# mrankitvish/ai-agent-kubectl

Measured on AMD Instinct MI355X. Metric: requests/sec + p50 e2e latency, /kubectl-command Llama-3-8B 1/2/4/8 GPU, higher is better.
Workload: dtype bf16; 1 GPU; model=Llama-3-8B-Instruct, global_batch=256, seq_len=115, parallelism=dp1

## Files before the change

ai_agent_kubectl_amd/csrc/attention.hip:

```cpp
#include "common.h"

#define HD 128
#define KBS 16


struct DecodeFuse {
  const bf16_t* qkv;
  const float* P;
  int split;
  int pbf16;
  size_t pstride;
  const int* positions;
  const float* cos_sin;
  const int* slot_mapping;
  bf16_t* k_cache;
  bf16_t* v_cache;
  const int* nshared;
  bf16_t* q_out;
  float* part_o;
  float* part_ml;
};

constexpr int DQ_UNROLL = 4;
template <int N>
__device__ __forceinline__ void dq_ld4n(const DecodeFuse& f, const size_t (&off)[N], const bool (&en)[N],
                                        uint2 (&out)[N]) {
  if (f.P == nullptr) {
#pragma unroll
    for (int n = 0; n < N; ++n)
      if (en[n]) out[n] = *reinterpret_cast<const uint2*>(f.qkv + off[n]);
    return;
  }
  f32x4 s[N];
#pragma unroll
  for (int n = 0; n < N; ++n) s[n] = f32x4{0.f, 0.f, 0.f, 0.f};
  if (f.pbf16) {
    const bf16_t* pb = reinterpret_cast<const bf16_t*>(f.P);
    for (int k0 = 0; k0 < f.split; k0 += DQ_UNROLL) {
      uint2 q[DQ_UNROLL][N];
#pragma unroll
      for (int k = 0; k < DQ_UNROLL; ++k)
#pragma unroll
        for (int n = 0; n < N; ++n)
          if (en[n] && k0 + k < f.split) q[k][n] = *reinterpret_cast<const uint2*>(pb + (k0 + k) * f.pstride + off[n]);
#pragma unroll
      for (int k = 0; k < DQ_UNROLL; ++k)
#pragma unroll
        for (int n = 0; n < N; ++n)
          if (en[n] && k0 + k < f.split) s[n] += f32x4{lo_f(q[k][n].x), hi_f(q[k][n].x), lo_f(q[k][n].y), hi_f(q[k][n].y)};
    }
  } else {
    constexpr int U = DQ_UNROLL / 2;
    for (int k0 = 0; k0 < f.split; k0 += U) {
      f32x4 p[U][N];
#pragma unroll
      for (int k = 0; k < U; ++k)
#pragma unroll
        for (int n = 0; n < N; ++n)
          if (en[n] && k0 + k < f.split) p[k][n] = *reinterpret_cast<const f32x4*>(f.P + (k0 + k) * f.pstride + off[n]);
#pragma unroll
      for (int k = 0; k < U; ++k)
#pragma unroll
        for (int n = 0; n < N; ++n)
          if (en[n] && k0 + k < f.split) s[n] += p[k][n];
    }
  }
#pragma unroll
  for (int n = 0; n < N; ++n) out[n] = make_uint2(pack2(s[n][0], s[n][1]), pack2(s[n][2], s[n][3]));
}

template <bool FUSED, int NW = 4>
__global__ __launch_bounds__(64 * NW, 4) void paged_decode_kernel(bf16_t* __restrict__ out, const bf16_t* __restrict__ q,
                                                           const bf16_t* __restrict__ k_cache,
                                                           const bf16_t* __restrict__ v_cache,
                                                           const int* __restrict__ block_tables, int max_blocks,
                                                           const int* __restrict__ ctx_lens, int hq, int hkv,
                                                           float scale_log2, DecodeFuse fz) {
  const int h = blockIdx.x, b = blockIdx.y;
  const int G = hq / hkv;
  const int lane = threadIdx.x & 63, wave = FUSED ? __builtin_amdgcn_readfirstlane(threadIdx.x >> 6) : threadIdx.x >> 6;
  const int col = lane & 15, grp = lane >> 4;
  int ns = 0;
  int pos_b = 0, slot_b = -1;
// ... 537 lines not shown
    l[r] = 0.f;
  }
#pragma unroll
  for (int n = 0; n < 8; ++n) o[n] = f32x4{0.f, 0.f, 0.f, 0.f};

  u32x4 kreg[2], vreg[2];
  prefill_load_tile(kreg, vreg, k_cache, v_cache, bt, nblocks, 0, h, hkv);
  bf16_t* pw = s.p[wave];
  for (int t = 0; t < ntiles; ++t) {
    __syncthreads();
    prefill_store_tile(s, kreg, vreg);
    __syncthreads();
    if (t + 1 < ntiles) prefill_load_tile(kreg, vreg, k_cache, v_cache, bt, nblocks, t + 1, h, hkv);
    const int t0 = t * 32;
    f32x4 sc[2];
#pragma unroll
    for (int j = 0; j < 2; ++j) {
      const int tok = 16 * j + col;
      f32x4 acc = {0.f, 0.f, 0.f, 0.f};
#pragma unroll
      for (int ks = 0; ks < 4; ++ks) {
        const uint4 kf = s.k[tok][(4 * ks + grp) ^ (tok & 15)];
        acc = mfma16x16x32(qf[ks], as_bf16x8(kf), acc);
      }
      sc[j] = acc;
    }
    float alpha[4];
#pragma unroll
    for (int r = 0; r < 4; ++r) {
      const float x0 = (t0 + col <= qpos[r]) ? sc[0][r] * scale_log2 : -INFINITY;
      const float x1 = (t0 + 16 + col <= qpos[r]) ? sc[1][r] * scale_log2 : -INFINITY;
      const float mx = row16_max(fmaxf(x0, x1));
      const float mn = fmaxf(m[r], mx);
      alpha[r] = (mn == -INFINITY) ? 1.f : exp2f(m[r] - mn);
      const float p0 = (mn == -INFINITY) ? 0.f : exp2f(x0 - mn);
      const float p1 = (mn == -INFINITY) ? 0.f : exp2f(x1 - mn);
      l[r] = l[r] * alpha[r] + row16_sum(p0 + p1);
      m[r] = mn;
      p_store(pw, 4 * grp + r, col, p0, p1);
    }
#pragma unroll
    for (int n = 0; n < 8; ++n) {
#pragma unroll
      for (int r = 0; r < 4; ++r) o[n][r] *= alpha[r];
    }
    asm volatile("s_waitcnt lgkmcnt(0)" ::: "memory");
    const bf16x8 pf = p_load(pw, col, grp);
#pragma unroll
    for (int n = 0; n < 8; ++n) {
      const int dim = n * 16 + col;
      const uint4 vf = s.v[dim][grp ^ (((dim >> 2) & 1) << 1)];
      o[n] = mfma16x16x32(pf, as_bf16x8(vf), o[n]);
    }
  }
#pragma unroll
  for (int r = 0; r < 4; ++r) {
    const int row = wave * 16 + 4 * grp + r;
    const int tok = tile_tok0 + row / G;
    const int g = row % G;
    if (tok >= qlen) continue;
    const float inv = l[r] > 0.f ? 1.f / l[r] : 0.f;
    bf16_t* op = out + ((size_t)(q0 + tok) * hq + h * G + g) * HD + col;
#pragma unroll
    for (int n = 0; n < 8; ++n) op[n * 16] = f2bf(o[n][r] * inv);
  }
}

extern "C" int ka_paged_prefill(void* out, const void* q, const void* k_cache, const void* v_cache,
                                const int* block_tables, int max_blocks, const int* q_starts, const int* ctx_lens,
                                int num_seqs, int max_q_len, int hq, int hkv, int head_dim, int block_size,
                                float scale, hipStream_t stream) {
  if (num_seqs <= 0 || max_q_len <= 0) return 0;
  const int G = hkv > 0 ? hq / hkv : 0;
  if (head_dim != HD || block_size != KBS || hq % hkv != 0 || G > 64 || 64 % G != 0) return (int)hipErrorInvalidValue;
  const float scale_log2 = scale * 1.4426950408889634f;
  const int tpt = 64 / G;
  const int qtiles = (max_q_len + tpt - 1) / tpt;
  hipLaunchKernelGGL(paged_prefill_kernel, dim3(qtiles, hkv, num_seqs), dim3(256), 0, stream,
                     static_cast<bf16_t*>(out), static_cast<const bf16_t*>(q), static_cast<const bf16_t*>(k_cache),
                     static_cast<const bf16_t*>(v_cache), block_tables, max_blocks, q_starts, ctx_lens, hq, hkv,
                     scale_log2);
  KA_CHECK_LAUNCH();
}
```

ai_agent_kubectl_amd/models/llama.py:

```python
from __future__ import annotations

import os
from dataclasses import dataclass
from typing import Dict, Optional

import torch
import torch.nn.functional as F

from .. import ops
from ..parallel.comm import LocalComm
from .config import ModelConfig
from .moe import moe_forward


def persistent_default() -> bool:
    mode = os.environ.get("KA_PERSISTENT_DECODE", "auto")
    if mode in ("0", "1"):
        return mode == "1"
    return float(os.environ.get("KA_GPU_MEM_SHARE", "1")) >= 1.0


@dataclass
class AttnMeta:
    positions: torch.Tensor
    slot_mapping: torch.Tensor
    block_tables: torch.Tensor
    ctx_lens: torch.Tensor
    logits_indices: torch.Tensor
    is_decode: bool
    q_starts: Optional[torch.Tensor] = None
    max_q_len: int = 1
    num_decode: int = 0
    num_tokens: int = 0
    shared_blocks: Optional[torch.Tensor] = None


SAMP_WORDS = 6


@dataclass
class SampleArrays:
    temperature: torch.Tensor
    top_k: torch.Tensor
    top_p: torch.Tensor
    seed: torch.Tensor
    position: torch.Tensor

    @classmethod
    def from_image(cls, img: torch.Tensor, cap: int, n: int) -> "SampleArrays":
        return cls(temperature=img[0:n].view(torch.float32), top_k=img[cap:cap + n],
                   top_p=img[2 * cap:2 * cap + n].view(torch.float32), position=img[3 * cap:3 * cap + n],
                   seed=img[4 * cap:4 * cap + 2 * n].view(torch.int64))


class LlamaModel:
    def __init__(self, cfg: ModelConfig, weights: Dict[str, torch.Tensor], comm=None, tp_rank: int = 0,
                 tp_size: int = 1, ep_rank: int = 0, ep_size: int = 1):
        self.cfg = cfg
        self.W = weights
        self.comm = comm or LocalComm()
        self.tp_rank, self.tp_size = tp_rank, tp_size
        self._local_comm = isinstance(self.comm, LocalComm)
        self.ep_rank, self.ep_size = ep_rank, ep_size
        self.hq = cfg.num_heads // tp_size
        self.hkv = cfg.num_kv_heads // tp_size
        self.D = cfg.head_dim
        self.scale = cfg.head_dim ** -0.5
        self.vocab_local = weights["lm_head"].shape[0]
        self.vocab_offset = tp_rank * self.vocab_local
        dev = weights["embed"].device
        self.device = dev
        self.cos_sin = ops.rope_cos_sin(cfg.max_position, cfg.head_dim, cfg.rope_theta, device=dev)
        self.fuse_decode_rope = os.environ.get("KA_FUSE_DECODE_ROPE", "1") == "1"
        self.bf16_partials = os.environ.get("KA_BF16_PARTIALS", "1") == "1"
        self.bf16_qkv_partials = os.environ.get("KA_BF16_QKV_PARTIALS", "1") == "1"
        self.layers = [self._layer(i) for i in range(cfg.num_layers)]
        w13 = self.layers[0].get("w13") if self.layers else None
        self.i_local = w13.shape[-2] // 2 if w13 is not None else cfg.intermediate // tp_size
        self.prune_last_layer = os.environ.get("KA_PRUNE_LAST_LAYER", "1") == "1"
        self.mark_layer = -1
        self.mark_event = None
        self.prefetch_bytes = int(float(os.environ.get("KA_DECODE_PREFETCH_MB", "0")) * (1 << 20))
        self.prefetch_max_b = int(os.environ.get("KA_DECODE_PREFETCH_MAX_B", "4"))
        self.prefetch_blocks = int(os.environ.get("KA_DECODE_PREFETCH_BLOCKS", "64"))
        self._side = None
        self.persistent = persistent_default()
        self._pd = None
        self.persistent_max_b = int(os.environ.get("KA_PERSISTENT_MAX_B", "2"))
        self._pd_max_b = None
        self.persistent_stamps = None

    def _layer(self, i):
        p = f"layers.{i}."
        return {k: self.W[p + k] for k in ("wqkv", "wo", "ln1", "ln2", "w13", "w2", "router") if p + k in self.W}

    def forward(self, input_ids: torch.Tensor, meta: AttnMeta, k_cache: torch.Tensor,
                v_cache: torch.Tensor) -> torch.Tensor:
        cfg = self.cfg
        eps = cfg.norm_eps
        h = ops.embedding(input_ids, self.W["embed"])
        if ops.reference_fp32():
            h = h.float()
        if meta.is_decode and not ops._ref(h) and self.persistent_ok(input_ids.shape[0]):
            return self._forward_persistent(h, meta, k_cache, v_cache)
        residual = None
        pending = False
        T = input_ids.shape[0]
        mark = self.mark_layer
        last_li = len(self.layers) - 1
        pruned = False
        for li, L in enumerate(self.layers):
            if li == mark and input_ids.is_cuda:
                self.mark_event = torch.cuda.Event()
                self.mark_event.record()
            if residual is None:
                residual = h
                x = ops.rmsnorm(h, L["ln1"], eps)
            else:
                x = self._reduce_norm(h, L["ln1"], eps, residual, pending)
            fused = meta.is_decode and self.fuse_decode_rope
            qkv = ops.linear(x, L["wqkv"], defer_reduce=True, bf16_partials=fused and self.bf16_qkv_partials)
            side = self._fork_prefetch(L, T) if meta.is_decode else None
            if fused:
                a = ops.decode_attention_rope(qkv, meta.positions, self.cos_sin, meta.slot_mapping, k_cache[li],
                                              v_cache[li], meta.block_tables, meta.ctx_lens, self.hq, self.hkv,
                                              self.D, self.scale, shared_blocks=meta.shared_blocks)
            else:
                q = ops.rope_kv_write(qkv, meta.positions, self.cos_sin, meta.slot_mapping, k_cache[li],
                                      v_cache[li], self.hq, self.hkv, self.D)
                if li == last_li and not meta.is_decode and self.prune_last_layer:
                    idx = meta.logits_indices
                    a = ops.attention_decode(q.index_select(0, idx), k_cache[li], v_cache[li], meta.block_tables,
                                             meta.ctx_lens, self.scale)
                    residual = residual.index_select(0, idx)
                    pruned = True
                else:
                    a = self._attention(q, meta, k_cache[li], v_cache[li])
            if 0 < meta.num_tokens < T and not meta.is_decode and not pruned:
                a[meta.num_tokens:].zero_()
            fuse = self._local_comm or (meta.is_decode and getattr(self.comm, "splitk_norm", False))
            h = ops.linear(a.reshape(a.shape[0], self.hq * self.D), L["wo"], defer_reduce=fuse,
                           bf16_partials=self.bf16_partials)
            x = self._reduce_norm(h, L["ln2"], eps, residual, True)
            if side is not None:
                torch.cuda.current_stream(self.device).wait_stream(side)
            combined = False
            if cfg.is_moe:
                h, combined = moe_forward(x, L, cfg, self.ep_rank, self.ep_size, meta.is_decode, self.comm)
            elif ops.use_prefill_swiglu(x, L["w13"]):
                h = ops.linear(ops.linear_swiglu(x, L["w13"]), L["w2"], defer_reduce=fuse,
                               bf16_partials=self.bf16_partials)
            elif sw := ops.decode_swiglu_cfg(x, L["w13"]):
                h = ops.linear(ops.linear_gm_swiglu(x, L["w13"], sw), L["w2"], defer_reduce=fuse,
                               bf16_partials=self.bf16_partials)
            else:
                h = ops.swiglu_linear(ops.linear(x, L["w13"], defer_reduce=True), L["w2"], defer_reduce=fuse,
                                      bf16_partials=self.bf16_partials)
            pending = not combined
        if meta.is_decode:
            return self._reduce_norm(h, self.W["norm"], eps, residual, pending)
        if pending and not self._local_comm:
            self.comm.all_reduce(h)
        if pruned:
            return ops.rmsnorm(h, self.W["norm"], eps, residual=residual)
        if isinstance(h, ops.SplitK):
            x = ops.rmsnorm(h, self.W["norm"], eps, residual=residual)
            return x.index_select(0, meta.logits_indices)
        idx = meta.logits_indices
        return ops.rmsnorm(h.index_select(0, idx), self.W["norm"], eps, residual=residual.index_select(0, idx))

    def persistent_ok(self, B: int = 1) -> bool:
        cfg = self.cfg
        comm_ok = (self._local_comm or getattr(self.comm, "persistent_no_reduce", False)
                   or self._tp_exchange() is not None)
        I = self.i_local
        if not (self.persistent and self.device.type == "cuda" and comm_ok and not cfg.is_moe
                and self.D == 128 and self.hq % self.hkv == 0 and self.hq // self.hkv <= 8
                and cfg.hidden % 512 == 0 and I % 512 == 0 and (self.hq * self.D) % 512 == 0
                and cfg.hidden <= 16384 and 1 <= B <= self.persistent_max_b):
            return False
        if self._pd_max_b is None:
            self._pd_max_b = ops.decode_persistent_max_b(cfg.hidden, self.hq, I, self.hq // self.hkv)
        return B <= self._pd_max_b

    def _tp_exchange(self):
        car = getattr(self.comm, "custom_ar", None)
        if car is None or self.tp_size <= 1 or os.environ.get("KA_PERSISTENT_TP", "0") != "1":
            return None
        return car.pd_exchange()

    def _forward_persistent(self, h0, meta: AttnMeta, k_cache, v_cache) -> torch.Tensor:
        if self._pd is None:
            ptrs = [[L[k].data_ptr() for k in ("wqkv", "wo", "w13", "w2", "ln1", "ln2")] for L in self.layers]
            table = torch.tensor(ptrs, dtype=torch.int64, device=self.device)
            lib = ops._hip.require()
            ws = torch.zeros(int(lib.ka_decode_persistent_ws(self.cfg.hidden, self.hq, self.hkv, self.i_local)),
                             dtype=torch.uint8, device=self.device)
            self._pd = (table, ws)
        table, ws = self._pd
        assert k_cache.shape[3] == 16, "persistent decode needs KV block 16"
        hout = ops.decode_persistent(h0, table, len(self.layers), self.hq, self.hkv, self.i_local,
                                     self.cfg.norm_eps, self.scale, k_cache, v_cache, meta.positions,
                                     meta.slot_mapping, meta.block_tables, meta.ctx_lens, self.cos_sin, ws,
                                     self.persistent_stamps, tp=self._tp_exchange())
        return ops.rmsnorm(hout, self.W["norm"], self.cfg.norm_eps)

    def persistent_err_word(self) -> Optional[torch.Tensor]:
        if self._pd is None:
            return None
        off = int(ops._hip.require().ka_decode_persistent_err_offset())
        return self._pd[1][off:off + 4].view(torch.int32)

    def persistent_err(self) -> int:
        if self._pd is None:
            return 0
        return int(ops._hip.require().ka_decode_persistent_err(self._pd[1].data_ptr(), ops._stream()))

    def _fork_prefetch(self, L, T: int):
        if not self.prefetch_bytes or T > self.prefetch_max_b or not self.device.type == "cuda" or "w13" not in L:
            return None
        if self._side is None:
# ... 47 lines not shown
```

ai_agent_kubectl_amd/ops/__init__.py:

```python
from __future__ import annotations

import bisect
import os
from typing import NamedTuple, Optional, Tuple

import torch

from . import reference as ref
from ._hip import check, require


_FORCE_REF = False
_REF_FP32 = False


class force_reference:

    def __init__(self, fp32: bool = False):
        self.fp32 = fp32

    def __enter__(self):
        global _FORCE_REF, _REF_FP32
        self._old = (_FORCE_REF, _REF_FP32)
        _FORCE_REF, _REF_FP32 = True, self.fp32
# ... 94 lines not shown
        return q_out
    if _ref(qkv):
        return ref.rope_kv_write(qkv, positions, cos_sin, slot_mapping, k_cache, v_cache, hq, hkv, d)
    lib = require()
    T = qkv.shape[0]
    q_out = torch.empty((T, hq, d), dtype=qkv.dtype, device=qkv.device) if q_out is None else q_out
    check(lib.ka_rope_kv(_p(q_out), _p(k_cache), _p(v_cache), _p(qkv), _p(positions), _p(cos_sin),
                         _p(slot_mapping), T, hq, hkv, d, k_cache.shape[2], _stream()), "rope_kv")
    return q_out


def attention_prefill(q, k_cache, v_cache, block_tables, q_starts, ctx_lens, max_q_len: int, scale: float,
                      out: Optional[torch.Tensor] = None) -> torch.Tensor:
    if _ref(q):
        r = ref.attention_prefill(q, k_cache, v_cache, block_tables, q_starts, ctx_lens, scale)
        if out is None:
            return r
        for i in range(ctx_lens.shape[0]):
            out[int(q_starts[i]):int(q_starts[i + 1])] = r[int(q_starts[i]):int(q_starts[i + 1])]
        return out
    lib = require()
    out = torch.empty_like(q) if out is None else out
    S = ctx_lens.shape[0]
    check(lib.ka_paged_prefill(_p(out), _p(q), _p(k_cache), _p(v_cache), _p(block_tables), block_tables.shape[1],
                               _p(q_starts), _p(ctx_lens), S, int(max_q_len), q.shape[1], k_cache.shape[1],
                               q.shape[2], k_cache.shape[2], float(scale), _stream()), "paged_prefill")
    return out


def attention_decode(q, k_cache, v_cache, block_tables, ctx_lens, scale: float,
                     out: Optional[torch.Tensor] = None) -> torch.Tensor:
    if _ref(q):
        r = ref.attention_decode(q, k_cache, v_cache, block_tables, ctx_lens, scale)
        if out is None:
            return r
        out.copy_(r)
        return out
    lib = require()
    out = torch.empty_like(q) if out is None else out
    check(lib.ka_paged_decode(_p(out), _p(q), _p(k_cache), _p(v_cache), _p(block_tables), block_tables.shape[1],
                              _p(ctx_lens), q.shape[0], q.shape[1], k_cache.shape[1], q.shape[2], k_cache.shape[2],
                              float(scale), _stream()), "paged_decode")
    return out


_CASCADE_WS = {}


def cascade_ok(B: int, hq: int, hkv: int) -> bool:
    g = hq // hkv
    return hq % hkv == 0 and g in (1, 2, 4, 8)


def decode_attention_rope(qkv, positions, cos_sin, slot_mapping, k_cache, v_cache, block_tables, ctx_lens,
                          hq: int, hkv: int, d: int, scale: float, out: Optional[torch.Tensor] = None,
                          shared_blocks: Optional[torch.Tensor] = None) -> torch.Tensor:
    lead = qkv.P if isinstance(qkv, SplitK) else qkv
    if _ref(lead) or d != 128 or k_cache.shape[2] != 16 or hq % hkv or hq // hkv > 15:
        if isinstance(qkv, SplitK) and qkv.is_bf16:
            qkv = qkv.resolve()
        q = rope_kv_write(qkv, positions, cos_sin, slot_mapping, k_cache, v_cache, hq, hkv, d)
        return attention_decode(q, k_cache, v_cache, block_tables, ctx_lens, scale, out=out)
    lib = require()
    B = ctx_lens.shape[0]
    out = torch.empty((B, hq, d), dtype=k_cache.dtype, device=k_cache.device) if out is None else out
    if isinstance(qkv, SplitK):
        src, P, split, pb = None, _p(qkv.P), qkv.split, int(qkv.is_bf16)
    else:
        src, P, split, pb = _p(qkv), None, 1, 0
    if shared_blocks is not None and cascade_ok(B, hq, hkv):
        key = (k_cache.device, B, hq)
        ws = _CASCADE_WS.get(key)
        if ws is None:
            ws = torch.empty(int(lib.ka_decode_cascade_ws(B, hq)), dtype=torch.uint8, device=k_cache.device)
            _CASCADE_WS[key] = ws
        check(lib.ka_paged_decode_rope_cascade(_p(out), src, P, split, pb, _p(k_cache), _p(v_cache), _p(positions),
                                               _p(cos_sin), _p(slot_mapping), _p(block_tables), block_tables.shape[1],
                                               _p(ctx_lens), B, hq, hkv, d, k_cache.shape[2], float(scale),
                                               _p(shared_blocks), _p(ws), _stream()), "paged_decode_rope_cascade")
        return out
    check(lib.ka_paged_decode_rope(_p(out), src, P, split, pb, _p(k_cache), _p(v_cache), _p(positions), _p(cos_sin),
                                   _p(slot_mapping), _p(block_tables), block_tables.shape[1], _p(ctx_lens), B, hq,
                                   hkv, d, k_cache.shape[2], float(scale), _stream()), "paged_decode_rope")
    return out


def silu_mul(gu, out: Optional[torch.Tensor] = None) -> torch.Tensor:
    if isinstance(gu, SplitK):
        lib = require()
        gu = gu.fp32()
        T, two_i = gu.shape
        out = torch.empty((T, two_i // 2), dtype=torch.bfloat16, device=gu.P.device) if out is None else out
        check(lib.ka_silu_mul_splitk(_p(out), _p(gu.P), gu.split, T, two_i // 2, _stream()), "silu_mul_splitk")
        return out
    if _ref(gu):
        return ref.silu_mul(gu)
    lib = require()
    T, two_i = gu.shape
    out = torch.empty((T, two_i // 2), dtype=gu.dtype, device=gu.device) if out is None else out
    check(lib.ka_silu_mul(_p(out), _p(gu), T, two_i // 2, _stream()), "silu_mul")
    return out


def prefetch(t: torch.Tensor, nbytes: int = 0, blocks: int = 0) -> None:
    if _ref(t):
        return
    lib = require()
    n = t.numel() * t.element_size()
    n = min(n, nbytes) if nbytes > 0 else n
    check(lib.ka_prefetch(_p(t), n, int(blocks), None, _stream()), "prefetch")


def embedding(ids: torch.Tensor, table: torch.Tensor, vocab_offset: int = 0,
              out: Optional[torch.Tensor] = None) -> torch.Tensor:
    if _ref(table):
        return ref.embedding(ids, table, vocab_offset)
    lib = require()
    T = ids.shape[0]
    out = torch.empty((T, table.shape[1]), dtype=table.dtype, device=table.device) if out is None else out
    check(lib.ka_embedding(_p(out), _p(ids), _p(table), T, table.shape[1], table.shape[0], int(vocab_offset),
                           _stream()), "embedding")
    return out


def masked_argmax(logits: torch.Tensor, mask_bits: Optional[torch.Tensor], mask_idx: Optional[torch.Tensor],
                  vocab_offset: int = 0, out_idx: Optional[torch.Tensor] = None,
                  out_val: Optional[torch.Tensor] = None) -> Tuple[torch.Tensor, torch.Tensor]:
    if _ref(logits):
        return ref.masked_argmax(logits, mask_bits, mask_idx, vocab_offset)
    lib = require()
    B, V = logits.shape
    out_idx = torch.empty(B, dtype=torch.int32, device=logits.device) if out_idx is None else out_idx
    out_val = torch.empty(B, dtype=torch.float32, device=logits.device) if out_val is None else out_val
    words = mask_bits.shape[1] if mask_bits is not None else 0
    slices = lib.ka_argmax_slices(B, V)
    ws = torch.empty(2 * B * slices, dtype=torch.float32, device=logits.device) if slices > 1 else None
    check(lib.ka_masked_argmax(_p(out_idx), _p(out_val), _p(logits), _p(mask_bits),
                               _p(mask_idx) if mask_bits is not None else None, B, V, words, int(vocab_offset),
                               _p(ws), slices, _stream()), "masked_argmax")
    return out_idx, out_val


def sample(logits: torch.Tensor, mask_bits: Optional[torch.Tensor], mask_idx: Optional[torch.Tensor],
           temperature: torch.Tensor, top_k: torch.Tensor, top_p: torch.Tensor, seed: torch.Tensor,
           position: torch.Tensor, vocab_offset: int = 0, return_cut: bool = False):
    if _ref(logits):
        return ref.sample(logits, mask_bits, mask_idx, temperature, top_k, top_p, seed, position, vocab_offset,
                          return_cut=return_cut)
    lib = require()
    B, V = logits.shape
    dev = logits.device
    for name, t, dt in (("temperature", temperature, torch.float32), ("top_k", top_k, torch.int32),
                        ("top_p", top_p, torch.float32), ("seed", seed, torch.int64),
                        ("position", position, torch.int32)):
        if t is None or t.dtype != dt or t.shape != (B,) or t.device != dev or not t.is_contiguous():
            raise ValueError(f"sample: {name} must be a contiguous {dt} [{B}] tensor on {dev}")
    if not logits.is_contiguous() or logits.dtype != torch.bfloat16:
        raise ValueError("sample: logits must be contiguous bf16 [rows, vocab]")
    out_idx = torch.empty(B, dtype=torch.int32, device=dev)
    out_val = torch.empty(B, dtype=torch.float32, device=dev)
    cut = torch.empty(B, dtype=torch.float32, device=dev) if return_cut else None
    kept = torch.empty(B, dtype=torch.int32, device=dev) if return_cut else None
    words = mask_bits.shape[1] if mask_bits is not None else 0
    slices = lib.ka_argmax_slices(B, V)
    ws = (torch.empty(lib.ka_sample_ws_words(B, slices), dtype=torch.int32, device=dev) if slices > 1 else None)
    check(lib.ka_sample(_p(out_idx), _p(out_val), _p(cut), _p(kept), _p(logits), _p(mask_bits),
# ... 528 lines not shown
```

ai_agent_kubectl_amd/ops/_hip.py:

```python
from __future__ import annotations

import ctypes
import os
import threading
from typing import Optional

LIB_DIR = os.path.join(os.path.dirname(os.path.abspath(__file__)), "lib")
DEFAULT_LIB = os.path.join(LIB_DIR, "libkagent_hip.so")


def _lib_path() -> str:
    alt = os.environ.get("KA_HIP_LIB")
    if alt and os.environ.get("KA_HIP_LIB_DIAG") == "1":
        return alt
    if alt:
        raise RuntimeError("KA_HIP_LIB is set without KA_HIP_LIB_DIAG=1: refusing to load a non-default "
                           f"kernel library ({alt}); unset it, or set KA_HIP_LIB_DIAG=1 for a diagnostic run")
    return DEFAULT_LIB


LIB_PATH = _lib_path()

_lock = threading.Lock()
_lib: Optional[ctypes.CDLL] = None
_err: Optional[str] = None

P = ctypes.c_void_p
I = ctypes.c_int
F = ctypes.c_float

_RESTYPES = {"ka_gemm_big_ws_bytes": ctypes.c_size_t, "ka_decode_persistent_ws": ctypes.c_size_t,
             "ka_decode_persistent_xbytes": ctypes.c_size_t, "ka_decode_persistent_xflag_offset": ctypes.c_size_t,
             "ka_decode_cascade_ws": ctypes.c_size_t}

_SIGS = {
    "ka_rmsnorm": [P, P, P, P, I, I, F, P],
    "ka_rope_kv": [P, P, P, P, P, P, P, I, I, I, I, I, P],
    "ka_silu_mul": [P, P, I, I, P],
    "ka_embedding": [P, P, P, I, I, I, I, P],
    "ka_masked_argmax": [P, P, P, P, P, I, I, I, I, P, I, P],
    "ka_argmax_slices": [I, I],
    "ka_sample": [P, P, P, P, P, P, P, P, P, P, P, P, I, I, I, I, P, I, P],
    "ka_sample_ws_words": [I, I],
    "ka_moe_topk": [P, P, P, I, I, I, P],
    "ka_paged_decode": [P, P, P, P, P, I, P, I, I, I, I, I, F, P],
    "ka_paged_decode_rope": [P, P, P, I, I, P, P, P, P, P, P, I, P, I, I, I, I, I, F, P],
    "ka_paged_decode_rope_cascade": [P, P, P, I, I, P, P, P, P, P, P, I, P, I, I, I, I, I, F, P, P, P],
    "ka_decode_cascade_ws": [I, I],
    "ka_paged_prefill": [P, P, P, P, P, I, P, P, I, I, I, I, I, I, F, P],
    "ka_gemm_skinny": [P, P, P, P, I, I, I, I, P],
    "ka_gemv_swiglu": [P, P, P, P, I, I, I, I, P],
    "ka_rmsnorm_splitk": [P, P, P, I, I, P, I, I, F, P],
    "ka_rope_kv_splitk": [P, P, P, P, I, P, P, P, I, I, I, I, I, P],
    "ka_silu_mul_splitk": [P, P, I, I, I, P],
    "ka_kv_block_copy": [P, P, P, P, I, I, ctypes.c_long, ctypes.c_long, P],
    "ka_prefetch": [P, ctypes.c_long, I, P, P],
    "ka_gemm_mfma": [P, P, P, P, I, I, I, I, I, I, I, I, I, P],
    "ka_gemv_rows": [P, P, P, P, I, I, I, I, I, I, P],
    "ka_gemm_mfma_swiglu": [P, P, P, I, I, I, I, I, I, P],
    "ka_gemm_mfma_grouped": [P, P, P, P, P, P, I, I, I, I, I, I, I, I, I, I, I, P],
    "ka_gemm_big": [P, P, P, P, I, I, I, I, I, I, I, P, ctypes.c_size_t, P],
    "ka_gemm_big_ws_bytes": [],
    "ka_gemm_big_plan": [I, I, I, I, ctypes.c_size_t, P, P],
    "ka_gemm_big_tn": [I, I, I],
    "ka_gemm_big_grouped": [P, P, P, P, I, P, I, I, I, I, I, I, I, P],
    "ka_gemm_big_err": [P, P],
    "ka_gemm_big_argmax": [P, P, P, P, I, I, I, I, P, P, I, I, P, P],
    "ka_argmax_finish": [P, P, P, P, I, I, I, P],
    "ka_argmax_combine": [P, P, P, I, I, P],
    "ka_decode_persistent": [P, P, P, I, I, I, I, I, F, F, P, P, ctypes.c_long, P, P, P, P, P, P, P, I, I, P],
    "ka_decode_persistent_tp": [P, P, P, I, I, I, I, I, F, F, P, P, ctypes.c_long, P, P, P, P, P, P, P, I, I, I, I,
                                P, P, P, P],
    "ka_decode_persistent_xbytes": [],
    "ka_decode_persistent_xflag_offset": [],
    "ka_decode_persistent_max_b": [I, I, I],
    "ka_decode_persistent_max_b2": [I, I, I, I],
    "ka_decode_persistent_ws": [I, I, I, I],
    "ka_decode_persistent_err": [P, P],
    "ka_decode_persistent_err_offset": [],
    "ka_gm_bn": [I],
    "ka_gm_bm": [I],
    "ka_moe_align": [P, P, P, I, I, I, P],
    "ka_moe_gemm": [P, P, P, P, P, I, I, I, I, I, I, I, P, P],
    "ka_moe_combine": [P, P, P, I, P, P, I, I, I, I, I, P],
    "ka_moe_sort": [P, P, P, P, P, P, I, I, I, I, I, P],
    "ka_allreduce_oneshot": [P, P, P, P, P, P, P, I, I, I, I, I, P],
    "ka_allgather_oneshot": [P, P, P, P, P, P, P, I, I, I, I, I, P],
    "ka_allreduce_rmsnorm": [P, P, P, P, F, P, P, P, P, P, I, I, I, I, I, I, I, I, P],
    "ka_ar_alloc": [P, ctypes.c_size_t],
    "ka_ar_free": [P],
    "ka_ar_get_handle": [P, P],
    "ka_ar_open_handle": [P, P],
    "ka_ar_close_handle": [P],
}


def load(path: str = LIB_PATH) -> Optional[ctypes.CDLL]:
    global _lib, _err
    with _lock:
        if _lib is not None:
            return _lib
        if not os.path.exists(path):
            _err = f"HIP kernel library not built: {path} (run python -c 'import __graft_entry__ as g; g.build()')"
            return None
        try:
            lib = ctypes.CDLL(path, mode=ctypes.RTLD_GLOBAL)
        except OSError as e:
            _err = f"failed to load {path}: {e}"
            return None
        for name, argtypes in _SIGS.items():
            fn = getattr(lib, name, None)
            if fn is None:
                continue
            fn.argtypes = argtypes
            fn.restype = _RESTYPES.get(name, ctypes.c_int)
        _lib = lib
        return _lib


def require() -> ctypes.CDLL:
    lib = load()
    if lib is None:
        raise RuntimeError(_err or "HIP kernel library unavailable")
    return lib


def available() -> bool:
    return load() is not None


def check(code: int, what: str) -> None:
    if code != 0:
# ... 2 lines not shown
```

Baseline: 1388 req/s.

## Fuse RoPE, KV-cache write and pad zeroing into paged prefill attention

Adds a paged prefill attention kernel that reads Q/K/V straight from the QKV projection output. It applies RoPE in registers, takes the new-token K/V from the activations rather than the cache, and writes the rotated K and the V into the paged cache from the first q-tile. Extra grid slices zero the padding rows, so a separate rope_kv_write kernel and a zero_ launch are no longer needed per prefill layer. The cost is a much more complex kernel: the KV-cache write is serialised in qt==0 workgroups, and the partial-tile/DPP V-transpose paths are easy to get wrong.

```diff
diff --git a/ai_agent_kubectl_amd/csrc/attention.hip b/ai_agent_kubectl_amd/csrc/attention.hip
--- a/ai_agent_kubectl_amd/csrc/attention.hip
+++ b/ai_agent_kubectl_amd/csrc/attention.hip
@@ -1,4 +1,6 @@
 #include "common.h"
+
+#include <algorithm>
 
 #define HD 128
 #define KBS 16
@@ -702,3 +704,360 @@
                      scale_log2);
   KA_CHECK_LAUNCH();
 }
+
+struct PrefillFuse {
+  const bf16_t* qkv;
+  const int* positions;
+  const float* cos_sin;
+  const int* slot_mapping;
+  bf16_t* k_cache;
+  bf16_t* v_cache;
+  int num_seqs;
+  int num_tokens;
+  int total_tokens;
+};
+
+KA_DEV void rope8(const uint4& a, const uint4& b, const float4& c0, const float4& c1, const float4& s0,
+                  const float4& s1, uint4& r1, uint4& r2) {
+  const uint32_t aw[4] = {a.x, a.y, a.z, a.w}, bw[4] = {b.x, b.y, b.z, b.w};
+  const float cc[8] = {c0.x, c0.y, c0.z, c0.w, c1.x, c1.y, c1.z, c1.w};
+  const float ss[8] = {s0.x, s0.y, s0.z, s0.w, s1.x, s1.y, s1.z, s1.w};
+  uint32_t o1[4], o2[4];
+  {
+#pragma clang fp contract(off)
+#pragma unroll
+    for (int k = 0; k < 4; ++k) {
+      const float xa0 = lo_f(aw[k]), xa1 = hi_f(aw[k]), xb0 = lo_f(bw[k]), xb1 = hi_f(bw[k]);
+      const float n0 = xb0 * ss[2 * k], n1 = xb1 * ss[2 * k + 1], p0 = xa0 * ss[2 * k], p1 = xa1 * ss[2 * k + 1];
+      o1[k] = pack2(__builtin_fmaf(xa0, cc[2 * k], -n0), __builtin_fmaf(xa1, cc[2 * k + 1], -n1));
+      o2[k] = pack2(__builtin_fmaf(xb0, cc[2 * k], p0), __builtin_fmaf(xb1, cc[2 * k + 1], p1));
+    }
+  }
+  r1 = make_uint4(o1[0], o1[1], o1[2], o1[3]);
+  r2 = make_uint4(o2[0], o2[1], o2[2], o2[3]);
+}
+
+KA_DEV uint4 rope_chunk(const uint4& own, const uint4& partner, int ch, const float4& c0, const float4& c1,
+                        const float4& s0, const float4& s1) {
+  const bool first = ch < 8;
+  uint4 r1, r2;
+  rope8(first ? own : partner, first ? partner : own, c0, c1, s0, s1, r1, r2);
+  return first ? r1 : r2;
+}
+
+KA_DEV uint32_t bf16_elem(const uint4& v, int k) {
+  const uint32_t w = (k >> 1) == 0 ? v.x : (k >> 1) == 1 ? v.y : (k >> 1) == 2 ? v.z : v.w;
+  return (k & 1) ? w >> 16 : w & 0xffffu;
+}
+
+__global__ __launch_bounds__(256, 3) void paged_prefill_rope_kernel(bf16_t* __restrict__ out,
+                                                                 const bf16_t* k_cache, const bf16_t* v_cache,
+                                                                 const int* __restrict__ block_tables, int max_blocks,
+                                                                 const int* __restrict__ q_starts,
+                                                                 const int* __restrict__ ctx_lens, int hq, int hkv,
+                                                                 float scale_log2, PrefillFuse fz) {
+  const int qt = blockIdx.x, h = blockIdx.y, sq = blockIdx.z;
+  const int tid = threadIdx.x;
+  if (sq >= fz.num_seqs) {
+    const size_t first = (size_t)fz.num_tokens * hq * (HD / 8);
+    const size_t end = (size_t)fz.total_tokens * hq * (HD / 8);
+    const size_t wg = ((size_t)(sq - fz.num_seqs) * gridDim.y + h) * gridDim.x + qt;
+    const size_t step = (size_t)(gridDim.z - fz.num_seqs) * gridDim.y * gridDim.x * 256;
+    for (size_t i = first + wg * 256 + tid; i < end; i += step)
+      reinterpret_cast<uint4*>(out)[i] = make_uint4(0, 0, 0, 0);
+    return;
+  }
+  const int G = hq / hkv;
+  const int tpt = 64 / G;
+  const int q0 = q_starts[sq];
+  const int qlen = q_starts[sq + 1] - q0;
+  const int tile_tok0 = qt * tpt;
+  if (tile_tok0 >= qlen) return;
+  const int ctx = ctx_lens[sq];
+  const int base_pos = ctx - qlen;
+  const int last_tok = min(tile_tok0 + tpt, qlen) - 1;
+  const int kv_end = base_pos + last_tok + 1;
+  const int ntiles = (kv_end + 31) >> 5;
+  const int nblocks = (ctx + KBS - 1) / KBS;
+  const int* bt = block_tables + (size_t)sq * max_blocks;
+  const size_t qstride = (size_t)(hq + 2 * hkv) * HD;
+  const size_t head_stride = (size_t)KBS * HD;
+
+  const int lane = tid & 63, wave = tid >> 6;
+  const int col = lane & 15, grp = lane >> 4;
+  __shared__ PrefillSmem s;
+
+  bf16x8 qf[4];
+  {
+    const int row = wave * 16 + col;
+    const int tok = tile_tok0 + row / G;
+    const int g = row % G;
+    if (tok < qlen) {
+      const bf16_t* qp = fz.qkv + (size_t)(q0 + tok) * qstride + (size_t)(h * G + g) * HD + 8 * grp;
+      const float* cs = fz.cos_sin + (size_t)fz.positions[q0 + tok] * HD + 8 * grp;
+      uint4 x[4];
+#pragma unroll
+      for (int ks = 0; ks < 4; ++ks) x[ks] = *reinterpret_cast<const uint4*>(qp + 32 * ks);
+#pragma unroll
+      for (int kk = 0; kk < 2; ++kk) {
+        const float* c = cs + 32 * kk;
+        uint4 r1, r2;
+        rope8(x[kk], x[kk + 2], *reinterpret_cast<const float4*>(c), *reinterpret_cast<const float4*>(c + 4),
+              *reinterpret_cast<const float4*>(c + HD / 2), *reinterpret_cast<const float4*>(c + HD / 2 + 4), r1, r2);
+        qf[kk] = as_bf16x8(r1);
+        qf[kk + 2] = as_bf16x8(r2);
+      }
+    } else {
+#pragma unroll
+      for (int ks = 0; ks < 4; ++ks) qf[ks] = as_bf16x8(make_uint4(0, 0, 0, 0));
+    }
+  }
+  int qpos[4];
+#pragma unroll
+  for (int r = 0; r < 4; ++r) {
+    const int row = wave * 16 + 4 * grp + r;
+    const int tok = tile_tok0 + row / G;
+    qpos[r] = tok < qlen ? base_pos + tok : kv_end - 1;
+  }
+  float m[4], l[4];
+  f32x4 o[8];
+#pragma unroll
+  for (int r = 0; r < 4; ++r) {
+    m[r] = -INFINITY;
+    l[r] = 0.f;
+  }
+#pragma unroll
+  for (int n = 0; n < 8; ++n) o[n] = f32x4{0.f, 0.f, 0.f, 0.f};
+
+  const int kt = tid >> 3, kc = tid & 7;
+  const int vt = tid & 31, vc = tid >> 5;
+  u32x4 kreg[2], vreg[2];
+  uint4 nv[2];
+  float4 ncs[4];
+  auto load_cache = [&](int tile) {
+    const int t0 = tile * 32;
+    if (t0 >= base_pos) return;
+    const int i0 = 2 * tile < nblocks ? 2 * tile : 0, i1 = 2 * tile + 1 < nblocks ? 2 * tile + 1 : 0;
+    const int blk0 = bt[__builtin_amdgcn_readfirstlane(i0)], blk1 = bt[__builtin_amdgcn_readfirstlane(i1)];
+    if (t0 + kt < base_pos) {
+      const bf16_t* kp = k_cache + ((size_t)((kt >> 4) ? blk1 : blk0) * hkv + h) * head_stride + (kt & 15) * HD + kc * 8;
+      kreg[0] = *reinterpret_cast<const u32x4*>(kp);
+      kreg[1] = *reinterpret_cast<const u32x4*>(kp + HD / 2);
+    }
+#pragma unroll
+    for (int i = 0; i < 2; ++i) {
+      const int p = tid + 256 * i;
+      const int dim = p >> 2, ch = p & 3;
+      const int blk = (ch >> 1) ? blk1 : blk0;
+      if (t0 + ch * 8 < base_pos)
+        vreg[i] = *reinterpret_cast<const u32x4*>(v_cache + ((size_t)blk * hkv + h) * head_stride + dim * KBS + (ch & 1) * 8);
+    }
+  };
+  auto load_new = [&](int tile) {
+    const int t0 = tile * 32;
+    if (t0 + 32 <= base_pos) return;
+    const int kpos = t0 + kt, vpos = t0 + vt;
+    if (kpos >= base_pos && kpos < ctx) {
+      const int t = q0 + kpos - base_pos;
+      const bf16_t* kp = fz.qkv + (size_t)t * qstride + (size_t)(hq + h) * HD + kc * 8;
+      kreg[0] = *reinterpret_cast<const u32x4*>(kp);
+      kreg[1] = *reinterpret_cast<const u32x4*>(kp + HD / 2);
+      const float* cs = fz.cos_sin + (size_t)fz.positions[t] * HD + kc * 8;
+      ncs[0] = *reinterpret_cast<const float4*>(cs);
+      ncs[1] = *reinterpret_cast<const float4*>(cs + 4);
+      ncs[2] = *reinterpret_cast<const float4*>(cs + HD / 2);
+      ncs[3] = *reinterpret_cast<const float4*>(cs + HD / 2 + 4);
+    }
+    if (vpos >= base_pos && vpos < ctx) {
+      const bf16_t* vp = fz.qkv + (size_t)(q0 + vpos - base_pos) * qstride + (size_t)(hq + hkv + h) * HD + vc * 8;
+      nv[0] = *reinterpret_cast<const uint4*>(vp);
+      nv[1] = *reinterpret_cast<const uint4*>(vp + HD / 2);
+    }
+  };
+  auto store_tile = [&](int tile) {
+    const int t0 = tile * 32;
+    {
+      const int kpos = t0 + kt;
+      uint4 k0 = __builtin_bit_cast(uint4, kreg[0]), k1 = __builtin_bit_cast(uint4, kreg[1]);
+      if (kpos >= base_pos) {
+        if (kpos < ctx) rope8(uint4(k0), uint4(k1), ncs[0], ncs[1], ncs[2], ncs[3], k0, k1);
+        else k0 = k1 = make_uint4(0, 0, 0, 0);
+      }
+      s.k[kt][kc ^ (kt & 15)] = k0;
+      s.k[kt][(kc + 8) ^ (kt & 15)] = k1;
+    }
+    if (t0 < base_pos) {
+#pragma unroll
+      for (int i = 0; i < 2; ++i) {
+        const int p = tid + 256 * i;
+        const int dim = p >> 2, ch = p & 3;
+        const int c0 = t0 + ch * 8;
+        uint4* dst = &s.v[dim][ch ^ (((dim >> 2) & 1) << 1)];
+        if (c0 + 8 <= base_pos) {
+          *reinterpret_cast<u32x4*>(dst) = vreg[i];
+        } else if (c0 < base_pos) {
+          const uint4 v = __builtin_bit_cast(uint4, vreg[i]);
+#pragma unroll
+          for (int k = 0; k < 7; ++k)
+            if (c0 + k < base_pos) reinterpret_cast<bf16_t*>(dst)[k] = (bf16_t)bf16_elem(v, k);
+        }
+      }
+    }
+    if (t0 + 32 > base_pos) {
+      const int vpos = t0 + vt;
+      const bool live = vpos >= base_pos && vpos < ctx;
+      const uint4 a0 = live ? nv[0] : make_uint4(0, 0, 0, 0), a1 = live ? nv[1] : make_uint4(0, 0, 0, 0);
+      const bool even = (vt & 1) == 0;
+      const uint4 give = even ? a1 : a0;
+      uint4 got;
+      got.x = __builtin_amdgcn_mov_dpp((int)give.x, 0xB1, 0xF, 0xF, false);
+      got.y = __builtin_amdgcn_mov_dpp((int)give.y, 0xB1, 0xF, 0xF, false);
+      got.z = __builtin_amdgcn_mov_dpp((int)give.z, 0xB1, 0xF, 0xF, false);
+      got.w = __builtin_amdgcn_mov_dpp((int)give.w, 0xB1, 0xF, 0xF, false);
+      const uint4 lo = even ? a0 : got, hi = even ? got : a1;
+      const int chunk = even ? vc : vc + 8;
+      const int pt = vt & ~1, pos0 = t0 + pt;
+      const int vchunk = pt >> 3, vword = (pt & 7) >> 1;
+      if (pos0 >= base_pos) {
+#pragma unroll
+        for (int k = 0; k < 8; ++k) {
+          const int dim = chunk * 8 + k;
+          reinterpret_cast<uint32_t*>(&s.v[dim][vchunk ^ (((dim >> 2) & 1) << 1)])[vword] =
+              bf16_elem(lo, k) | (bf16_elem(hi, k) << 16);
+        }
+      } else if (pos0 + 1 >= base_pos) {
+#pragma unroll
+        for (int k = 0; k < 8; ++k) {
+          const int dim = chunk * 8 + k;
+          reinterpret_cast<bf16_t*>(&s.v[dim][vchunk ^ (((dim >> 2) & 1) << 1)])[2 * vword + 1] = (bf16_t)bf16_elem(hi, k);
+        }
+      }
+    }
+  };
+  auto load_tile = [&](int tile) {
+    load_cache(tile);
+    load_new(tile);
+  };
+
+  load_tile(0);
+  bf16_t* pw = s.p[wave];
+  for (int t = 0; t < ntiles; ++t) {
+    __syncthreads();
+    store_tile(t);
+    __syncthreads();
+    if (t + 1 < ntiles) load_tile(t + 1);
+    const int t0 = t * 32;
+    f32x4 sc[2];
+#pragma unroll
+    for (int j = 0; j < 2; ++j) {
+      const int tok = 16 * j + col;
+      f32x4 acc = {0.f, 0.f, 0.f, 0.f};
+#pragma unroll
+      for (int ks = 0; ks < 4; ++ks) {
+        const uint4 kf = s.k[tok][(4 * ks + grp) ^ (tok & 15)];
+        acc = mfma16x16x32(qf[ks], as_bf16x8(kf), acc);
+      }
+      sc[j] = acc;
+    }
+    float alpha[4];
+#pragma unroll
+    for (int r = 0; r < 4; ++r) {
+      const float x0 = (t0 + col <= qpos[r]) ? sc[0][r] * scale_log2 : -INFINITY;
+      const float x1 = (t0 + 16 + col <= qpos[r]) ? sc[1][r] * scale_log2 : -INFINITY;
+      const float mx = row16_max(fmaxf(x0, x1));
+      const float mn = fmaxf(m[r], mx);
+      alpha[r] = (mn == -INFINITY) ? 1.f : exp2f(m[r] - mn);
+      const float p0 = (mn == -INFINITY) ? 0.f : exp2f(x0 - mn);
+      const float p1 = (mn == -INFINITY) ? 0.f : exp2f(x1 - mn);
+      l[r] = l[r] * alpha[r] + row16_sum(p0 + p1);
+      m[r] = mn;
+      p_store(pw, 4 * grp + r, col, p0, p1);
+    }
+#pragma unroll
+    for (int n = 0; n < 8; ++n) {
+#pragma unroll
+      for (int r = 0; r < 4; ++r) o[n][r] *= alpha[r];
+    }
+    asm volatile("s_waitcnt lgkmcnt(0)" ::: "memory");
+    const bf16x8 pf = p_load(pw, col, grp);
+#pragma unroll
+    for (int n = 0; n < 8; ++n) {
+      const int dim = n * 16 + col;
+      const uint4 vf = s.v[dim][grp ^ (((dim >> 2) & 1) << 1)];
+      o[n] = mfma16x16x32(pf, as_bf16x8(vf), o[n]);
+    }
+  }
+#pragma unroll
+  for (int r = 0; r < 4; ++r) {
+    const int row = wave * 16 + 4 * grp + r;
+    const int tok = tile_tok0 + row / G;
+    const int g = row % G;
+    if (tok >= qlen) continue;
+    const float inv = l[r] > 0.f ? 1.f / l[r] : 0.f;
+    bf16_t* op = out + ((size_t)(q0 + tok) * hq + h * G + g) * HD + col;
+#pragma unroll
+    for (int n = 0; n < 8; ++n) op[n * 16] = f2bf(o[n][r] * inv);
+  }
+
+  if (qt != 0) return;
+  bf16_t(*vtr)[18] = reinterpret_cast<bf16_t(*)[18]>(&s.k[0][0]);
+  const int aj = tid >> 4, ach = tid & 15;
+  for (int w0 = 0; w0 < qlen; w0 += 16) {
+    __syncthreads();
+    if (w0 + aj < qlen) {
+      const int t = q0 + w0 + aj;
+      const int slot = fz.slot_mapping[t];
+      const bf16_t* row = fz.qkv + (size_t)t * qstride;
+      const uint4 v = *reinterpret_cast<const uint4*>(row + (size_t)(hq + hkv + h) * HD + ach * 8);
+#pragma unroll
+      for (int k = 0; k < 8; ++k) vtr[ach * 8 + k][aj] = (bf16_t)bf16_elem(v, k);
+      if (slot >= 0) {
+        const bf16_t* kp = row + (size_t)(hq + h) * HD;
+        const float* cs = fz.cos_sin + (size_t)fz.positions[t] * HD + (ach & 7) * 8;
+        const uint4 kk = rope_chunk(*reinterpret_cast<const uint4*>(kp + ach * 8),
+                                    *reinterpret_cast<const uint4*>(kp + (ach ^ 8) * 8), ach,
+                                    *reinterpret_cast<const float4*>(cs), *reinterpret_cast<const float4*>(cs + 4),
+                                    *reinterpret_cast<const float4*>(cs + HD / 2),
+                                    *reinterpret_cast<const float4*>(cs + HD / 2 + 4));
+        *reinterpret_cast<uint4*>(fz.k_cache + (((size_t)(slot / KBS) * hkv + h) * KBS + slot % KBS) * HD + ach * 8) = kk;
+      }
+    }
+    __syncthreads();
+    const int lj = tid & 15;
+    const int ls = w0 + lj < qlen ? fz.slot_mapping[q0 + w0 + lj] : -1;
+    if (ls >= 0) {
+      bf16_t* dst = fz.v_cache + ((size_t)(ls / KBS) * hkv + h) * head_stride + ls % KBS;
+#pragma unroll
+      for (int k = 0; k < 8; ++k) {
+        const int dim = (tid >> 4) + 16 * k;
+        dst[(size_t)dim * KBS] = vtr[dim][lj];
+      }
+    }
+  }
+}
+
+extern "C" int ka_paged_prefill_rope(void* out, const void* qkv, void* k_cache, void* v_cache, const int* positions,
+                                     const float* cos_sin, const int* slot_mapping, const int* block_tables,
+                                     int max_blocks, const int* q_starts, const int* ctx_lens, int num_seqs,
+                                     int max_q_len, int num_tokens, int total_tokens, int hq, int hkv, int head_dim,
+                                     int block_size, float scale, hipStream_t stream) {
+  const int G = hkv > 0 ? hq / hkv : 0;
+  if (head_dim != HD || block_size != KBS || G <= 0 || hq % hkv != 0 || G > 64 || 64 % G != 0 || num_seqs < 0 ||
+      num_tokens < 0)
+    return (int)hipErrorInvalidValue;
+  if (max_q_len <= 0) num_seqs = 0;
+  const int pad_rows = total_tokens > num_tokens ? total_tokens - num_tokens : 0;
+  if (num_seqs == 0 && pad_rows == 0) return 0;
+  const float scale_log2 = scale * 1.4426950408889634f;
+  const int tpt = 64 / G;
+  const int qtiles = num_seqs > 0 ? (max_q_len + tpt - 1) / tpt : 1;
+  const long pad_chunks = (long)pad_rows * hq * (HD / 8), per_slice = (long)qtiles * hkv * 256 * 4;
+  const int zslices = pad_rows ? (int)std::min<long>(8, (pad_chunks + per_slice - 1) / per_slice) : 0;
+  PrefillFuse fz{static_cast<const bf16_t*>(qkv), positions, cos_sin, slot_mapping, static_cast<bf16_t*>(k_cache),
+                 static_cast<bf16_t*>(v_cache), num_seqs, num_tokens, num_tokens + pad_rows};
+  hipLaunchKernelGGL(paged_prefill_rope_kernel, dim3(qtiles, hkv, num_seqs + zslices), dim3(256), 0, stream,
+                     static_cast<bf16_t*>(out), static_cast<const bf16_t*>(k_cache),
+                     static_cast<const bf16_t*>(v_cache), block_tables, max_blocks, q_starts, ctx_lens, hq, hkv,
+                     scale_log2, fz);
+  KA_CHECK_LAUNCH();
+}
diff --git a/ai_agent_kubectl_amd/models/llama.py b/ai_agent_kubectl_amd/models/llama.py
--- a/ai_agent_kubectl_amd/models/llama.py
+++ b/ai_agent_kubectl_amd/models/llama.py
@@ -72,6 +72,7 @@
         self.device = dev
         self.cos_sin = ops.rope_cos_sin(cfg.max_position, cfg.head_dim, cfg.rope_theta, device=dev)
         self.fuse_decode_rope = os.environ.get("KA_FUSE_DECODE_ROPE", "1") == "1"
+        self.fuse_prefill_rope = os.environ.get("KA_FUSE_PREFILL_ROPE", "1") == "1"
         self.bf16_partials = os.environ.get("KA_BF16_PARTIALS", "1") == "1"
         self.bf16_qkv_partials = os.environ.get("KA_BF16_QKV_PARTIALS", "1") == "1"
         self.layers = [self._layer(i) for i in range(cfg.num_layers)]
@@ -121,10 +122,18 @@
             fused = meta.is_decode and self.fuse_decode_rope
             qkv = ops.linear(x, L["wqkv"], defer_reduce=True, bf16_partials=fused and self.bf16_qkv_partials)
             side = self._fork_prefetch(L, T) if meta.is_decode else None
+            padded = False
             if fused:
                 a = ops.decode_attention_rope(qkv, meta.positions, self.cos_sin, meta.slot_mapping, k_cache[li],
                                               v_cache[li], meta.block_tables, meta.ctx_lens, self.hq, self.hkv,
                                               self.D, self.scale, shared_blocks=meta.shared_blocks)
+            elif (self.fuse_prefill_rope and not meta.is_decode and not isinstance(qkv, ops.SplitK)
+                  and not (li == last_li and self.prune_last_layer)):
+                a = ops.prefill_attention_rope(qkv, meta.positions, self.cos_sin, meta.slot_mapping, k_cache[li],
+                                               v_cache[li], meta.block_tables, meta.q_starts, meta.ctx_lens,
+                                               meta.max_q_len, self.hq, self.hkv, self.D, self.scale,
+                                               num_decode=meta.num_decode, num_tokens=meta.num_tokens)
+                padded = True
             else:
                 q = ops.rope_kv_write(qkv, meta.positions, self.cos_sin, meta.slot_mapping, k_cache[li],
                                       v_cache[li], self.hq, self.hkv, self.D)
@@ -136,7 +145,7 @@
                     pruned = True
                 else:
                     a = self._attention(q, meta, k_cache[li], v_cache[li])
-            if 0 < meta.num_tokens < T and not meta.is_decode and not pruned:
+            if 0 < meta.num_tokens < T and not meta.is_decode and not pruned and not padded:
                 a[meta.num_tokens:].zero_()
             fuse = self._local_comm or (meta.is_decode and getattr(self.comm, "splitk_norm", False))
             h = ops.linear(a.reshape(a.shape[0], self.hq * self.D), L["wo"], defer_reduce=fuse,
diff --git a/ai_agent_kubectl_amd/ops/__init__.py b/ai_agent_kubectl_amd/ops/__init__.py
--- a/ai_agent_kubectl_amd/ops/__init__.py
+++ b/ai_agent_kubectl_amd/ops/__init__.py
@@ -200,6 +200,37 @@
     check(lib.ka_paged_decode_rope(_p(out), src, P, split, pb, _p(k_cache), _p(v_cache), _p(positions), _p(cos_sin),
                                    _p(slot_mapping), _p(block_tables), block_tables.shape[1], _p(ctx_lens), B, hq,
                                    hkv, d, k_cache.shape[2], float(scale), _stream()), "paged_decode_rope")
+    return out
+
+
+def prefill_attention_rope(qkv, positions, cos_sin, slot_mapping, k_cache, v_cache, block_tables, q_starts, ctx_lens,
+                           max_q_len: int, hq: int, hkv: int, d: int, scale: float, num_decode: int = 0,
+                           num_tokens: int = 0, out: Optional[torch.Tensor] = None) -> torch.Tensor:
+    T = qkv.shape[0]
+    nd = int(num_decode)
+    ntok = int(num_tokens) if 0 < int(num_tokens) < T else T
+    S = ctx_lens.shape[0]
+    lead = qkv.P if isinstance(qkv, SplitK) else qkv
+    g = hq // hkv if hkv and hq % hkv == 0 else 0
+    if isinstance(qkv, SplitK) or _ref(lead) or d != 128 or k_cache.shape[2] != 16 or g not in (1, 2, 4, 8):
+        q = rope_kv_write(qkv, positions, cos_sin, slot_mapping, k_cache, v_cache, hq, hkv, d)
+        a = attention_prefill(q, k_cache, v_cache, block_tables[nd:], q_starts[nd:], ctx_lens[nd:], max_q_len, scale,
+                              out=torch.empty_like(q) if out is None and nd else out)
+        if nd:
+            attention_decode(q[:nd], k_cache, v_cache, block_tables[:nd], ctx_lens[:nd], scale, out=a[:nd])
+        if ntok < T:
+            a[ntok:].zero_()
+        return a
+    lib = require()
+    out = torch.empty((T, hq, d), dtype=qkv.dtype, device=qkv.device) if out is None else out
+    if nd:
+        decode_attention_rope(qkv[:nd], positions[:nd], cos_sin, slot_mapping[:nd], k_cache, v_cache, block_tables[:nd],
+                              ctx_lens[:nd], hq, hkv, d, scale, out=out[:nd])
+    bt = block_tables[nd:]
+    check(lib.ka_paged_prefill_rope(_p(out), _p(qkv), _p(k_cache), _p(v_cache), _p(positions), _p(cos_sin),
+                                    _p(slot_mapping), _p(bt), block_tables.shape[1], _p(q_starts[nd:]),
+                                    _p(ctx_lens[nd:]), S - nd, int(max_q_len), ntok, T, hq, hkv, d, k_cache.shape[2],
+                                    float(scale), _stream()), "paged_prefill_rope")
     return out
 
 
diff --git a/ai_agent_kubectl_amd/ops/_hip.py b/ai_agent_kubectl_amd/ops/_hip.py
--- a/ai_agent_kubectl_amd/ops/_hip.py
+++ b/ai_agent_kubectl_amd/ops/_hip.py
@@ -48,6 +48,7 @@
     "ka_paged_decode_rope_cascade": [P, P, P, I, I, P, P, P, P, P, P, I, P, I, I, I, I, I, F, P, P, P],
     "ka_decode_cascade_ws": [I, I],
     "ka_paged_prefill": [P, P, P, P, P, I, P, P, I, I, I, I, I, I, F, P],
+    "ka_paged_prefill_rope": [P, P, P, P, P, P, P, P, I, P, P, I, I, I, I, I, I, I, I, F, P],
     "ka_gemm_skinny": [P, P, P, P, I, I, I, I, P],
     "ka_gemv_swiglu": [P, P, P, P, I, I, I, I, P],
     "ka_rmsnorm_splitk": [P, P, P, I, I, P, I, I, F, P],
```

Measured after the change: 1368 req/s. -1.4%, worse.
